# baldhat/yolov10-3D

Hardware: AMD Instinct MI355X
Metric: train_images_per_sec (higher is better)
Workload: dtype bf16

## Files before the change

### include/y3d.h

```cpp
#ifndef Y3D_H
#define Y3D_H
#include <stdint.h>

#ifdef __cplusplus
extern "C" {
#endif

enum { Y3D_F32 = 0, Y3D_BF16 = 1 };
enum { Y3D_OK = 0, Y3D_ERR_INVALID = -1, Y3D_ERR_HIP = -2 };

const char* y3d_last_error(void);
int y3d_abi_version(void);
int y3d_device_info(char* name, int name_len, int* compute_units, int* lds_bytes, int* clock_khz);

int y3d_pack_weight_fwd(int dtype, const float* w_oihw, void* out, int Cout, int Cin_g, int Cin_g_pad, int kh, int kw, void* stream);
int y3d_pack_weight_dgrad(int dtype, const float* w_oihw, void* out, int Cout, int Cin_g, int groups, int kh, int kw, void* stream);
int y3d_mt_pack_weights(int dtype, const int64_t* desc, const int* chunk_tensor, const int* chunk_off, int nchunks, int chunk, void* stream);
int y3d_mt_fp8w_quantize(const int64_t* desc, const int* row_begin, int ntensors, int nrows, void* stream);
int y3d_fp8w_dequantize(const uint8_t* codes, const float* scale, float* w, int rows, int K, void* stream);
int y3d_fp8_quantize_act(const void* x, int64_t xsw, int64_t M, int C, uint8_t* q, uint8_t* s, void* stream);
int y3d_fp8_pack_weight_fwd(const uint8_t* codes, const float* scale, int rows, int Cg, uint8_t* wq, uint8_t* ws, void* stream);
int y3d_conv3x3_fp8_ok(int B, int H, int W, int Cin, int Cout, int groups);
int y3d_conv3x3_fp8_stat_rows(int B, int H, int W);
int y3d_fp8_scale_pitch(int C);
// ... 13 lines not shown
  Y3D_ROUTE_GENERIC = 0,
  Y3D_ROUTE_STREAM1X1 = 1,
  Y3D_ROUTE_SMALL = 2,
  Y3D_ROUTE_SMALL_S2 = 3,
  Y3D_ROUTE_S2_DGRAD = 4,
  Y3D_ROUTE_TILE8 = 5,
  Y3D_ROUTE_TILE16 = 6,
  Y3D_ROUTE_WIDE3_8 = 7,
  Y3D_ROUTE_WIDE3_16 = 8,
  Y3D_ROUTE_FLAT = 9,
  Y3D_ROUTE_WGRAD_SMALL = 10,
  Y3D_ROUTE_WGRAD_TILE = 11,
  Y3D_ROUTE_WGRAD_STREAM1X1 = 12
};
int y3d_conv2d_route(int dtype, int op, int epi, int B, int H, int W, int Cin, int Cout, int groups, int kh, int kw, int stride, int pad);
int y3d_conv2d_fwd(int dtype, const void* x, int64_t xsb, int64_t xsh, int64_t xsw, int B, int H, int W, int Cin,
                   const void* w_packed, const float* bias, void* y, int64_t ysw, int Ho, int Wo, int Cout, int groups,
                   int kh, int kw, int stride, int pad, float* stat_partials, void* stream);
int y3d_conv2d_fwd_affine(int dtype, const void* x, int64_t xsb, int64_t xsh, int64_t xsw, int B, int H, int W, int Cin,
                          const void* w_packed, const float* scale, const float* shift, int act, void* y, int64_t ysw, int Ho, int Wo,
                          int Cout, int groups, int kh, int kw, int stride, int pad, void* stream);
int y3d_conv2d_fwd_affine_res_ok(int dtype, int B, int H, int W, int Cin, int Cout, int groups, int kh, int kw, int stride, int pad);
int y3d_conv2d_fwd_affine_res(int dtype, const void* x, int64_t xsb, int64_t xsh, int64_t xsw, int B, int H, int W, int Cin,
                              const void* w_packed, const float* scale, const float* shift, int act, const void* res, int64_t rsw, void* y,
                              int64_t ysw, int Ho, int Wo, int Cout, int groups, int kh, int kw, int stride, int pad, void* stream);
int y3d_conv2d_bwd_data(int dtype, const void* dy, int64_t dsb, int64_t dsh, int64_t dsw, int B, int Ho, int Wo, int Cout,
                        const void* w_packed_dgrad, void* dx, int64_t xsw, int H, int W, int Cin, int groups, int kh, int kw,
                        int stride, int pad, void* stream);
int y3d_conv2d_wgrad_splits(int dtype, int B, int Ho, int Wo, int Cout, int Cin_g, int groups, int kh, int kw);
int y3d_conv2d_wgrad_plan(int dtype, int B, int H, int W, int Cin, int Cout, int groups, int kh, int kw, int stride, int pad);
int y3d_set_tile_kernels(int enable);
int y3d_set_stream1x1(int enable);
int y3d_get_stream1x1(void);
int y3d_get_tile_kernels(void);
int y3d_set_bn_wide_slabs(int enable);
int y3d_conv2d_bwd_weight(int dtype, const void* x, int64_t xsb, int64_t xsh, int64_t xsw, int B, int H, int W, int Cin,
                          int Cin_real, const void* dy, int64_t dsw, int Ho, int Wo, int Cout, int groups, int kh, int kw,
                          int stride, int pad, float* slab, int nsplit, float* grad_oihw, int accumulate, void* stream);

int y3d_dw_blocks(int64_t M);
int y3d_dw_wgrad_blocks(int64_t M);
int y3d_dw_pack_weight(const float* w_oihw, float* out_taps_c, int C, int kh, int kw, void* stream);
int y3d_dwconv2d_fwd(int dtype, const void* x, int64_t xsb, int64_t xsh, int64_t xsw, int B, int H, int W, int C,
                     const float* w_packed, void* y, int64_t ysw, int Ho, int Wo, int kh, int kw, int stride, int pad,
                     float* stat_partials, void* stream);
int y3d_dwconv2d_fwd_affine(int dtype, const void* x, int64_t xsb, int64_t xsh, int64_t xsw, int B, int H, int W, int C,
                            const float* w_packed, const float* scale, const float* shift, int act, int res_mode, const void* res, int64_t rsw,
                            void* z, int64_t zsw, int Ho, int Wo, int kh, int kw, int stride, int pad, void* stream);
int y3d_dwconv2d_bwd_data(int dtype, const void* dy, int64_t dsb, int64_t dsh, int64_t dsw, int B, int Ho, int Wo, int C,
                          const float* w_packed, void* dx, int64_t xsw, int H, int W, int kh, int kw, int stride, int pad,
                          void* stream);
int y3d_dwconv2d_bwd_weight(int dtype, const void* x, int64_t xsb, int64_t xsh, int64_t xsw, int B, int H, int W, int C,
                            const void* dy, int64_t dsw, int Ho, int Wo, int kh, int kw, int stride, int pad, float* slab,
                            float* grad_oihw, int accumulate, void* stream);

int y3d_bn_finalize(const float* partials, int nblk, int C, int64_t count, const float* gamma, const float* beta, float eps,
                    float momentum, float* running_mean, float* running_var, float* mean, float* invstd, float* scale,
                    float* shift, void* stream);
int y3d_bn_eval_scale(int C, const float* gamma, const float* beta, const float* running_mean, const float* running_var,
                      float eps, float* scale, float* shift, void* stream);
int y3d_bn_act_fwd(int dtype, const void* y, int64_t ysw, const float* scale, const float* shift, int act, int res_mode,
                   const void* res, int64_t rsw, void* z, int64_t zsw, int64_t P, int C, void* stream);
int y3d_bn_act_fwd_q(const void* y, int64_t ysw, const float* scale, const float* shift, int act, void* z, int64_t zsw, uint8_t* q, uint8_t* s,
                     int64_t P, int C, void* stream);
int y3d_bn_bwd_blocks(int64_t P, int C);
int y3d_bn_act_bwd_reduce(int dtype, const void* y, int64_t ysw, const void* dz, int64_t dsw, const void* res, int64_t rsw,
// ... 192 lines not shown
```

### yolov10-3d_amd/_lib.py

```python
from __future__ import annotations

import ctypes
import os
import re

_HERE = os.path.dirname(os.path.abspath(__file__))
LIB_PATH = os.path.join(_HERE, "liby3d_hip.so")
HEADER = os.path.join(os.path.dirname(_HERE), "include", "y3d.h")

F32, BF16 = 0, 1

_CT = {"int": ctypes.c_int, "int64_t": ctypes.c_int64, "float": ctypes.c_float, "double": ctypes.c_double}


class Y3DError(RuntimeError):
    pass


def parse_header(path: str = HEADER):
    src = open(path).read()
    src = re.sub(r"/\*.*?\*/", " ", src, flags=re.S)
    protos = {}
    for m in re.finditer(r"(const\s+char\s*\*|int)\s+(y3d_\w+)\s*\(([^;{]*?)\)\s*;", src, flags=re.S):
        ret, name, args = m.group(1), m.group(2), m.group(3).strip()
        argtypes = []
        if args and args != "void":
            for a in args.split(","):
                a = a.strip()
                if "*" in a:
                    argtypes.append(ctypes.c_void_p)
                else:
                    toks = a.split()
                    t = toks[1] if toks[0] == "const" else toks[0]
                    argtypes.append(_CT[t])
        protos[name] = (ctypes.c_char_p if "char" in ret else ctypes.c_int, argtypes)
    return protos


_PLAIN_INT = {"abi_version", "conv_kpad", "conv_stat_blocks", "conv2d_stat_rows", "conv2d_route", "conv2d_wgrad_splits", "conv2d_wgrad_plan", "set_tile_kernels", "set_stream1x1", "set_bn_wide_slabs", "get_stream1x1", "get_tile_kernels", "dw_blocks", "dw_wgrad_blocks", "bn_bwd_blocks", "proj_blocks", "proj_group_blocks", "proj_group_bn_bwd_blocks", "proj_group_bwd_weight_bn_mfma_blocks", "tal3d_scratch_floats", "tal2d_scratch_floats", "v10_postprocess_scratch_floats", "conv2d_fwd_affine_res_ok", "stem_conv_train_rows", "conv3x3_fp8_ok", "conv3x3_fp8_dgrad_ok", "conv3x3_fp8_stat_rows", "fp8_scale_pitch", "kitti_eval_max_boxes", "det_metrics_max_gts", "det_metrics_max_dets"}


class _Lib:
    def __init__(self):
        if not os.path.exists(LIB_PATH):
            raise Y3DError(
                f"{LIB_PATH} not found: build it with `python yolov10-3d_amd/csrc/build.py` "
                "(or __graft_entry__.build()). There is no CPU / PyTorch fallback for the HIP path.")
        self._dll = ctypes.CDLL(LIB_PATH)
        self.protos = parse_header()
        for name, (ret, argtypes) in self.protos.items():
            fn = getattr(self._dll, name)
            fn.restype = ret
            fn.argtypes = argtypes

    def last_error(self) -> str:
        return (self._dll.y3d_last_error() or b"").decode()

    def __getattr__(self, name):
        if name.startswith("_"):
            raise AttributeError(name)
        fn = getattr(self._dll, "y3d_" + name)
        ret = self.protos["y3d_" + name][0]
        if ret is not ctypes.c_int or name in _PLAIN_INT:
            setattr(self, name, fn)
            return fn

        def call(*a):
            rc = fn(*a)
            if rc != 0:
                raise Y3DError(f"y3d_{name} failed ({rc}): {self.last_error()}")
            return rc

# ... 13 lines not shown
```

### yolov10-3d_amd/csrc/conv1x1_stream.hip

```cpp
#include "common.h"
#include "conv_frag.h"
#include <cstdlib>

namespace {

struct PwP {
  const bf16_t* x;
  const bf16_t* w;
  const float *bias, *scale, *shift;
  bf16_t* y;
  float* part;
  long ysw;
  int xsw;
  int M, K, N, Kpad;
  int nkc, nmt, nnt, act;
  int G, PC;
  unsigned xbytes, ybytes, pbytes, wbytes;
};

template <int N> __device__ __forceinline__ void pw_wvm() { asm volatile("s_waitcnt vmcnt(%0)" ::"n"(N) : "memory"); }
__device__ __forceinline__ void pw_wvm_n(int n) {
#define PW_C(i) case i: pw_wvm<i>(); break;
#define PW_C8(i) PW_C(i) PW_C(i + 1) PW_C(i + 2) PW_C(i + 3) PW_C(i + 4) PW_C(i + 5) PW_C(i + 6) PW_C(i + 7)
  switch (n) {
    PW_C8(0) PW_C8(8) PW_C8(16) PW_C8(24) PW_C8(32) PW_C8(40) PW_C8(48) PW_C(56) PW_C(57) PW_C(58) PW_C(59) PW_C(60) PW_C(61) PW_C(62)
    default: pw_wvm<63>(); break;
  }
#undef PW_C8
#undef PW_C
}
typedef __attribute__((ext_vector_type(2))) unsigned pw_u32x2;

template <int BN, int WP, int WC, int NS, bool AFF, bool WRES>
__global__ __launch_bounds__(512) void conv1x1_stream_kernel(PwP p) {
  {
    const int g = blockIdx.y;
    p.x += (long)g * p.K;
    p.w += (long)g * p.N * p.Kpad;
    p.y += (long)g * p.N;
    if (p.bias) p.bias += g * p.N;
    if (p.scale) { p.scale += g * p.N; p.shift += g * p.N; }
    if (p.part) p.part += (long)g * p.N * 2;
  }
  constexpr int BM = 128;
  constexpr int TP = BM / WP / 16, TC = BN / WC / 16;
  static_assert(WP * WC == 8 && TP >= 1 && TC >= 1, "8 waves");
  constexpr int STAGE = BM * 128 + (WRES ? 0 : BN * 128);
  constexpr int ND = 2 + (WRES ? 0 : BN / 64);
  static_assert(WRES || BN % 64 == 0, "streamed weight tiles: whole DMA instructions per wave");
  extern __shared__ __attribute__((aligned(16))) char smem[];
  char* sW = smem;
  char* sA = smem + (WRES ? (size_t)p.nkc * BN * 128 : 0);
  const int tid = threadIdx.x, lane = tid & 63, wave = __builtin_amdgcn_readfirstlane(tid >> 6);
  const int wp = wave % WP, wc = wave / WP;
  const int bid = blockIdx.x, xcd = bid & 7, idx = bid >> 3;
  const int nt = idx % p.nnt, wk = (idx / p.nnt) * 8 + xcd, nwk = (gridDim.x / p.nnt);
  const int n0 = nt * BN;
  const int mine = wk < p.nmt ? (p.nmt - wk + nwk - 1) / nwk : 0;
  const int S = mine * p.nkc;
  if (S == 0) {
    if (p.part && tid < BN && n0 + tid < p.N) *(float2*)(p.part + ((long)wk * p.PC + n0 + tid) * 2) = make_float2(0.f, 0.f);
    return;
  }

  if (WRES)
  for (int i = tid; i < p.nkc * BN * 8; i += 512) {
    const int c = i & 7, r = (i >> 3) % BN, kc = i / (8 * BN);
    const int k = kc * 64 + c * 8, n = n0 + r;
    uint4 v = make_uint4(0, 0, 0, 0);
    if (n < p.N && k < p.Kpad) v = *(const uint4*)(p.w + (long)n * p.Kpad + k);
    *(uint4*)(sW + (kc * BN + r) * 128 + ((c ^ (r & 7)) << 4)) = v;
  }

  const __amdgpu_buffer_rsrc_t rx = __builtin_amdgcn_make_buffer_rsrc((void*)p.x, 0, (int)p.xbytes, 0x00020000);
  const __amdgpu_buffer_rsrc_t rw = __builtin_amdgcn_make_buffer_rsrc((void*)p.w, 0, (int)p.wbytes, 0x00020000);
  constexpr unsigned OOB = 0xfffffff0u;
  const int lrow = lane >> 3, lchunk = (lane & 7) ^ lrow;
  int is = 0, i_tile = wk, i_kc = 0, i_slot = 0;
  auto issue = [&]() {
    const bool live = is < S;
    const int k = i_kc * 64 + lchunk * 8;
#pragma unroll
    for (int h = 0; h < 2; ++h) {
      const int r = 16 * wave + 8 * h;
      const int m = i_tile * BM + r + lrow;
      const bool ok = live & (m < p.M) & (k < p.K);
      const unsigned off = (unsigned)(m * p.xsw + k) * 2u;
      __builtin_amdgcn_raw_ptr_buffer_load_lds(rx, (__attribute__((address_space(3))) void*)(sA + i_slot * STAGE + r * 128), 16, ok ? off : OOB, 0, 0, 0);
    }
    if (!WRES) {
#pragma unroll
      for (int h = 0; h < BN / 64; ++h) {
        const int r = (BN / 8) * wave + 8 * h;
        const int n = n0 + r + lrow;
        const bool ok = live & (n < p.N) & (k < p.K);
        __builtin_amdgcn_raw_ptr_buffer_load_lds(rw, (__attribute__((address_space(3))) void*)(sA + i_slot * STAGE + (BM + r) * 128), 16,
                                                 ok ? (unsigned)(n * p.Kpad + k) * 2u : OOB, 0, 0, 0);
      }
    }
    ++is;
    if (++i_kc == p.nkc) { i_kc = 0; i_tile += nwk; }
    if (++i_slot == NS) i_slot = 0;
  };
#pragma unroll
  for (int s = 0; s < NS - 1; ++s) issue();

  f32x4_t acc[TC][TP];
  const int lc = (lane >> 4) * 4, lp = lane & 15;
  int c_tile = wk, c_kc = 0, c_slot = 0;
  int hist[NS - 1];
#pragma unroll
  for (int i = 0; i < NS - 1; ++i) hist[i] = 0;
  const __amdgpu_buffer_rsrc_t ry = __builtin_amdgcn_make_buffer_rsrc((void*)p.y, 0, (int)p.ybytes, 0x00020000);
  asm volatile("s_waitcnt lgkmcnt(0)" ::: "memory");

  float ssum[TC][4], ssq[TC][4];
#pragma unroll
  for (int a = 0; a < TC; ++a)
#pragma unroll
    for (int j = 0; j < 4; ++j) { ssum[a][j] = 0.f; ssq[a][j] = 0.f; }

#pragma unroll 1
  for (int s = 0; s < S; ++s) {
    {
      int young = ND * (NS - 2);
#pragma unroll
      for (int i = 0; i < NS - 1; ++i) young += hist[i];
      pw_wvm_n(young);
#pragma unroll
      for (int i = 0; i < NS - 2; ++i) hist[i] = hist[i + 1];
      hist[NS - 2] = 0;
    }
    __builtin_amdgcn_s_barrier();
    issue();
    if (c_kc == 0) {
#pragma unroll
      for (int a = 0; a < TC; ++a)
#pragma unroll
// ... 48 lines not shown
      }
    }
    hist[NS - 2] += TC * TP;
    c_tile += nwk;
  }
  pw_wvm<0>();
  if (p.part) {
    __syncthreads();
    float* red = (float*)sA;
#pragma unroll
    for (int a = 0; a < TC; ++a)
#pragma unroll
      for (int j = 0; j < 4; ++j) {
        const float s = wave_xor_sum16(ssum[a][j]), q = wave_xor_sum16(ssq[a][j]);
        if (lp == 0) {
          const int cl = wc * (BN / WC) + a * 16 + lc + j;
          red[(wp * BN + cl) * 2] = s;
          red[(wp * BN + cl) * 2 + 1] = q;
        }
      }
    __syncthreads();
    if (tid < BN && n0 + tid < p.N) {
      float s = 0.f, q = 0.f;
#pragma unroll
      for (int w = 0; w < WP; ++w) { s += red[(w * BN + tid) * 2]; q += red[(w * BN + tid) * 2 + 1]; }
      float* dst = p.part + ((long)wk * p.PC + n0 + tid) * 2;
      dst[0] = s;
      dst[1] = q;
    }
  }
}

struct PwPlan {
  int bn, ns, nnt, grid, wres;
  size_t lds;
};

bool pw_plan(int M, int K, int N, PwPlan* pl, int G = 1) {
  const int nkc = cdiv(K, 64);
  const size_t cap = 160 * 1024;
  const int nmt = cdiv(M, 128);
  const int bns[4] = {256, 128, 64, 32};
  int bn = 0;
  for (int i = 0; i < 4; ++i) {
    const int b = bns[i];
    if (i < 3 && bns[i + 1] >= N) continue;
    if ((size_t)b * nkc * 128 + 3 * 16384 <= cap) { bn = b; break; }
  }
  const bool can_stream = N > 64 && nkc >= 2;
  bool wres = bn != 0 && (cdiv(N, bn) == 1 || (cdiv(N, bn) == 2 && nmt < 200));
  if (!wres && !can_stream) {
    if (!bn) return false;
    wres = true;
  }
  pl->wres = wres;
  if (wres) {
    const size_t wb = (size_t)bn * nkc * 128;
    pl->bn = bn;
    pl->ns = wb + 4 * 16384 <= cap ? 4 : 3;
    pl->lds = wb + pl->ns * 16384;
  } else {
    pl->bn = N > 128 ? 256 : 128;
    pl->ns = pl->bn == 256 ? 3 : 4;
    pl->lds = (size_t)pl->ns * (16384 + pl->bn * 128);
  }
  pl->nnt = cdiv(N, pl->bn);
  const int per_cu = pl->lds <= 80 * 1024 ? 2 : 1;
  int wpx = (32 * per_cu) / (pl->nnt * G);
  if (wpx < 1) wpx = 1;
  if (wpx > cdiv(nmt, 8)) wpx = cdiv(nmt, 8);
  pl->grid = 8 * wpx * pl->nnt;
  return true;
}

template <int BN, int WP, int WC, int NS, bool AFF, bool WRES>
void pw_launch_1(const PwP& p, const PwPlan& pl, hipStream_t st) {
  static bool attr = false;
  if (!attr) {
    (void)hipFuncSetAttribute((const void*)conv1x1_stream_kernel<BN, WP, WC, NS, AFF, WRES>, hipFuncAttributeMaxDynamicSharedMemorySize, 160 * 1024);
    attr = true;
  }
  hipLaunchKernelGGL((conv1x1_stream_kernel<BN, WP, WC, NS, AFF, WRES>), dim3(pl.grid, p.G), dim3(512), pl.lds, st, p);
}

template <int BN, int WP, int WC>
void pw_launch_ns(const PwP& p, const PwPlan& pl, hipStream_t st) {
  const bool aff = p.bias || p.scale;
  if (pl.ns == 4) { if (aff) pw_launch_1<BN, WP, WC, 4, true, true>(p, pl, st); else pw_launch_1<BN, WP, WC, 4, false, true>(p, pl, st); }
  else { if (aff) pw_launch_1<BN, WP, WC, 3, true, true>(p, pl, st); else pw_launch_1<BN, WP, WC, 3, false, true>(p, pl, st); }
}

}

static int g_stream1x1 = 1;

extern "C" int y3d_get_stream1x1(void) { return g_stream1x1; }

extern "C" int y3d_set_stream1x1(int enable) {
  const int old = g_stream1x1;
  g_stream1x1 = enable ? 1 : 0;
  return old;
}

int y3d_conv1x1_stream_ok(int dtype, long M, int K, int N, long xsw, int G) {
  if (!g_stream1x1 || dtype != Y3D_BF16 || K % 8 != 0 || K < 32 || N < 8 || N % 4 != 0 || M < 128 || G < 1 || G > 64) return 0;
  if ((M * xsw + (long)G * K) * 2 >= (1L << 32) - 64 || M * N * G * 2 >= (1L << 31)) return 0;
  PwPlan pl;
  if (!pw_plan((int)M, K, N, &pl, G)) return 0;
  return 1;
}

int y3d_conv1x1_stream_rows(long M, int K, int N, int G) {
  PwPlan pl;
  if (!pw_plan((int)M, K, N, &pl, G)) return 0;
  return pl.grid / pl.nnt;
}

int y3d_conv1x1_stream_launch(const void* x, long xsw, const void* w, int Kpad, const float* bias, const float* scale, const float* shift, int act,
                              void* y, long ysw, float* part, long M, int K, int N, int G, void* stream) {
  PwPlan pl;
  Y3D_CHECK(pw_plan((int)M, K, N, &pl, G), "conv1x1_stream: no tile plan for K=%d N=%d", K, N);
  Y3D_CHECK(((uintptr_t)x & 15) == 0 && xsw % 8 == 0 && ((uintptr_t)w & 15) == 0 && Kpad % 8 == 0 && ((uintptr_t)y & 7) == 0 && ysw % 4 == 0,
            "conv1x1_stream: operand alignment");
  PwP p;
  p.x = (const bf16_t*)x; p.w = (const bf16_t*)w; p.bias = bias; p.scale = scale; p.shift = shift; p.y = (bf16_t*)y; p.part = part;
  p.ysw = ysw; p.xsw = (int)xsw; p.M = (int)M; p.K = K; p.N = N; p.Kpad = Kpad;
  p.nkc = cdiv(K, 64); p.nmt = cdiv(M, 128); p.nnt = pl.nnt; p.act = act; p.G = G; p.PC = G * N;
  p.xbytes = (unsigned)(((M - 1) * xsw + K) * 2);
  Y3D_CHECK(((M - 1) * ysw + (long)G * N) * 2 < (1L << 32) - 64 && M * ysw < (1L << 31), "conv1x1_stream: output tensor beyond 32-bit byte offsets");
  p.ybytes = (unsigned)(((M - 1) * ysw + N) * 2);
  p.pbytes = part ? (unsigned)((long)p.nmt * N * 8) : 0u;
  hipStream_t st = (hipStream_t)stream;
  p.wbytes = (unsigned)((long)N * Kpad * 2);
  if (!pl.wres) {
    const bool aff = bias || scale;
    if (pl.bn == 256) { if (aff) pw_launch_1<256, 2, 4, 3, true, false>(p, pl, st); else pw_launch_1<256, 2, 4, 3, false, false>(p, pl, st); }
    else { if (aff) pw_launch_1<128, 4, 2, 4, true, false>(p, pl, st); else pw_launch_1<128, 4, 2, 4, false, false>(p, pl, st); }
    Y3D_LAUNCH_CHECK();
    return Y3D_OK;
  }
  switch (pl.bn) {
    case 256: pw_launch_ns<256, 2, 4>(p, pl, st); break;
    case 128: pw_launch_ns<128, 4, 2>(p, pl, st); break;
    case 64: pw_launch_ns<64, 8, 1>(p, pl, st); break;
    default: pw_launch_ns<32, 8, 1>(p, pl, st); break;
  }
  Y3D_LAUNCH_CHECK();
  return Y3D_OK;
}
```

### yolov10-3d_amd/csrc/conv_gemm.hip

```cpp
#include "common.h"
#include "conv_frag.h"
#include <cstdlib>

namespace {

struct ConvP {
  const void* x;
  const void* w;
  const float* bias;
  const float* scale;
  const float* shift;
  int act;
  void* y;
  float* part;
  long xsb, xsh, xsw;
  long ysw;
  int B, Hg, Wg;
  int Hq, Wq;
  int Cg, Cn, G;
  int kh, kw, stride, pad;
  int Ktot, Kpad;
  int M;
  int ntx, nty;
};
// ... 635 lines not shown
    size_t sm = 2 * (128 + 64) * 128;
    hipLaunchKernelGGL((conv_gemm_kernel<T, 128, 64, 4, 1, MODE>), dim3(p.ntx * p.nty, ny, p.G), block, sm, st, p);
  } else {
    size_t sm = 2 * (128 + 32) * 128;
    hipLaunchKernelGGL((conv_gemm_kernel<T, 128, 32, 4, 1, MODE>), dim3(p.ntx * p.nty, ny, p.G), block, sm, st, p);
  }
  Y3D_LAUNCH_CHECK();
  return Y3D_OK;
}

template <typename T, bool DGRAD>
int launch_conv(ConvP p, hipStream_t st) {
  if (DGRAD && p.kh == 3 && p.kw == 3 && p.stride == 2 && p.pad == 1 && p.Cg % TT<T>::CE == 0) return launch_conv_mode<T, 2>(p, st);
  return launch_conv_mode<T, DGRAD ? 1 : 0>(p, st);
}

}

int y3d_conv3x3_tile_route(int dtype, int B, int H, int W, int Cg, int Cn, int G, int kh, int kw, int stride, int pad);
int y3d_conv3x3_flat_tiles(int B, int H, int W);
int y3d_conv3x3_tile_launch(int dtype, int route, const void* x, long xsb, long xsh, long xsw, int B, int H, int W, int Cg, int Cn, int G,
                            const void* w, int Ktot, void* y, long ysw, float* part, int flip, const float* scale, const float* shift, int act,
                            void* stream);

int y3d_wgrad_tile_height(int dtype, int H, int W, int Cg, int Cn, int kh, int kw, int stride, int pad);
int y3d_wgrad_tile_splits(int th, int B, int H, int W, int Cg, int Cn, int G);
int y3d_conv3x3_wgrad_tile_launch(int th, const void* x, long xsb, long xsh, long xsw, const void* dy, long dsw, int B, int H, int W, int Cg,
                                  int Cn, int G, float* slab, int nsplit, void* stream);

int y3d_conv1x1_stream_ok(int dtype, long M, int K, int N, long xsw, int G = 1);
int y3d_conv1x1_stream_launch(const void* x, long xsw, const void* w, int Kpad, const float* bias, const float* scale, const float* shift, int act,
                              void* y, long ysw, float* part, long M, int K, int N, int G, void* stream);
int y3d_wgrad1x1_stream_ok(int dtype, long M, int Cg, int Cn, long xsw, long dsw);
int y3d_wgrad1x1_stream_launch(const void* x, long xsw, const void* dy, long dsw, long M, int Cg, int Cn, float* slab, int nsplit, int chunk_px,
                               void* stream);
int y3d_conv3x3s2_dgrad_ok(int dtype, int B, int Ho, int Wo, int H, int W, int Cout, int Cin, long dsw, long xsw);
int y3d_conv3x3s2_dgrad_launch(const void* dy, long dsw, int B, int Ho, int Wo, int Cout, const void* w_packed_dgrad, int Kpad, void* dx, long xsw,
                               int H, int W, int Cin, void* stream);
int y3d_conv3x3_small_ok(int dtype, int B, int H, int W, int Cin, int Cout, int rows);
int y3d_conv3x3_small_launch(const void* x, long xsb, long xsh, long xsw, int B, int H, int W, int Cin, int Cout, const void* w, int Ktot, void* y,
                             long ysw, float* part, int rows, int flip, const float* scale, const float* shift, int act, const void* res, long rsw,
                             void* stream);
int y3d_conv3x3_small_rows(int B, int H, int W, int Cin, int Cout);
int y3d_conv3x3_small_s2_ok(int dtype, int B, int H, int W, int Cin, int Cout);
int y3d_conv3x3_small_s2_rows(int B, int H, int W, int Cin, int Cout);
int y3d_conv3x3_small_s2_launch(const void* x, long xsb, long xsh, long xsw, int B, int H, int W, int Cin, int Cout, const void* w, int Ktot, void* y,
                                long ysw, float* part, int rows, const float* scale, const float* shift, int act, void* stream);
int y3d_conv1x1_stream_rows(long M, int K, int N, int G = 1);
int y3d_wgrad3x3_small_ok(int dtype, int B, int H, int W, int Cin, int Cout);
int y3d_wgrad3x3_small_splits(int B, int H, int W);
int y3d_wgrad3x3_small_launch(const void* x, long xsb, long xsh, long xsw, const void* dy, long dsw, int B, int H, int W, int Cin, int Cout,
                              float* slab, int nsplit, void* stream);
static inline bool dense_pixels(int B, int H, int W, long sb, long sh, long sw) {
  return (H == 1 || sh == (long)W * sw) && (B == 1 || sb == (long)H * W * sw);
}

static int g_tile_kernels = 1;
extern "C" int y3d_conv2d_wgrad_splits(int dtype, int B, int Ho, int Wo, int Cout, int Cin_g, int groups, int kh, int kw);

static int conv_route(int dtype, int op, int epi, int B, int H, int W, int Ho, int Wo, int Cin, int Cout, int groups, int kh, int kw, int stride,
                      int pad, bool dense, long asw, long bsw, bool cin_full) {
  const int ce = dtype == Y3D_BF16 ? 8 : 4;
  const bool k1 = kh == 1 && kw == 1 && stride == 1 && pad == 0, k3s1 = kh == 3 && kw == 3 && stride == 1 && pad == 1,
             k3s2 = kh == 3 && kw == 3 && stride == 2 && pad == 1;
  if (op == Y3D_OP_FWD) {
    Y3D_CHECK(dtype == Y3D_BF16 || dtype == Y3D_F32, "conv2d_fwd: bad dtype %d", dtype);
// ... 35 lines not shown
  if (k3s1 && groups == 1 && cin_full && y3d_wgrad3x3_small_ok(dtype, B, H, W, Cin, Cout)) return Y3D_ROUTE_WGRAD_SMALL;
  if (g_tile_kernels && cin_full && y3d_wgrad_tile_height(dtype, H, W, Cin / groups, Cout / groups, kh, kw, stride, pad)) return Y3D_ROUTE_WGRAD_TILE;
  if (k1 && groups == 1 && cin_full && dense && y3d_wgrad1x1_stream_ok(dtype, (long)B * Ho * Wo, Cin, Cout, asw, bsw)) return Y3D_ROUTE_WGRAD_STREAM1X1;
  return Y3D_ROUTE_GENERIC;
}

extern "C" {

int y3d_get_tile_kernels(void) { return g_tile_kernels; }

int y3d_set_tile_kernels(int enable) {
  int old = g_tile_kernels;
  g_tile_kernels = enable ? 1 : 0;
  return old;
}

int y3d_conv_stat_blocks(int B, int Ho, int Wo) { return cdiv((long)B * Ho * Wo, 128); }

int y3d_conv2d_route(int dtype, int op, int epi, int B, int H, int W, int Cin, int Cout, int groups, int kh, int kw, int stride, int pad) {
  Y3D_CHECK(kh > 0 && kw > 0 && stride > 0 && pad >= 0, "conv2d_route: bad filter geometry");
  const int Ho = (H + 2 * pad - kh) / stride + 1, Wo = (W + 2 * pad - kw) / stride + 1;
  Y3D_CHECK(Ho > 0 && Wo > 0, "conv2d_route: empty output");
  if (op == Y3D_OP_BWD_DATA) return conv_route(dtype, op, epi, B, H, W, Ho, Wo, Cin, Cout, groups, kh, kw, stride, pad, true, Cout, Cin, true);
  return conv_route(dtype, op, epi, B, H, W, Ho, Wo, Cin, Cout, groups, kh, kw, stride, pad, true, Cin, Cout, true);
}

int y3d_conv2d_wgrad_plan(int dtype, int B, int H, int W, int Cin, int Cout, int groups, int kh, int kw, int stride, int pad) {
  int Ho = (H + 2 * pad - kh) / stride + 1, Wo = (W + 2 * pad - kw) / stride + 1;
  switch (conv_route(dtype, Y3D_OP_BWD_WEIGHT, 0, B, H, W, Ho, Wo, Cin, Cout, groups, kh, kw, stride, pad, true, Cin, Cout, true)) {
    case Y3D_ROUTE_WGRAD_SMALL: return y3d_wgrad3x3_small_splits(B, H, W);
    case Y3D_ROUTE_WGRAD_TILE:
      return y3d_wgrad_tile_splits(y3d_wgrad_tile_height(dtype, H, W, Cin / groups, Cout / groups, kh, kw, stride, pad), B, H, W, Cin / groups,
                                   Cout / groups, groups);
    case Y3D_ROUTE_WGRAD_STREAM1X1: {
      const int target = 256;
      const long tiles = (long)cdiv(Cin, Cin <= 64 ? 64 : 128) * cdiv(Cout, Cout <= 64 ? 64 : 128);
      long want = target / tiles, maxs = cdiv((long)B * H * W, 4 * 64);
      if (want > maxs) want = maxs;
      return (int)(want < 1 ? 1 : want);
    }
    default: return y3d_conv2d_wgrad_splits(dtype, B, Ho, Wo, Cout, Cin / groups, groups, kh, kw);
  }
}

int y3d_conv2d_stat_rows(int dtype, int B, int H, int W, int Cin, int Cout, int groups, int kh, int kw, int stride, int pad) {
  int Ho = (H + 2 * pad - kh) / stride + 1, Wo = (W + 2 * pad - kw) / stride + 1;
  switch (conv_route(dtype, Y3D_OP_FWD, Y3D_EPI_PARTIALS, B, H, W, Ho, Wo, Cin, Cout, groups, kh, kw, stride, pad, true, Cin, Cout, true)) {
    case Y3D_ROUTE_STREAM1X1: return y3d_conv1x1_stream_rows((long)B * H * W, Cin / groups, Cout / groups, groups);
    case Y3D_ROUTE_SMALL: return y3d_conv3x3_small_rows(B, H, W, Cin, Cout);
    case Y3D_ROUTE_SMALL_S2: return y3d_conv3x3_small_s2_rows(B, H, W, Cin, Cout);
    case Y3D_ROUTE_FLAT: return y3d_conv3x3_flat_tiles(B, H, W);
    case Y3D_ROUTE_TILE8: case Y3D_ROUTE_WIDE3_8: return B * cdiv(H, 8) * cdiv(W, 16);
    case Y3D_ROUTE_TILE16: case Y3D_ROUTE_WIDE3_16: return B * cdiv(H, 16) * cdiv(W, 16);
    default: return cdiv((long)B * Ho * Wo, 128);
  }
}

int y3d_conv_kpad(int dtype, int k_total) {
  int ce = dtype == Y3D_BF16 ? 8 : 4;
  return cdiv(k_total, ce) * ce;
}

int y3d_pack_weight_fwd(int dtype, const float* w_oihw, void* out, int Cout, int Cin_g, int Cin_g_pad, int kh, int kw, void* stream) {
  int ce = dtype == Y3D_BF16 ? 8 : 4;
  Y3D_CHECK(Cin_g_pad >= Cin_g && Cin_g_pad % ce == 0, "pack_weight_fwd: Cin_g_pad=%d must be a multiple of %d", Cin_g_pad, ce);
  int taps = kh * kw, Kpad = taps * Cin_g_pad;
  long n = (long)Cout * Kpad;
  hipStream_t st = (hipStream_t)stream;
  if (dtype == Y3D_BF16)
    hipLaunchKernelGGL(pack_w_fwd_kernel<bf16_t>, dim3(cdiv(n, 256)), dim3(256), 0, st, w_oihw, (bf16_t*)out, Cout, Cin_g, Cin_g_pad, taps, Kpad);
  else
    hipLaunchKernelGGL(pack_w_fwd_kernel<float>, dim3(cdiv(n, 256)), dim3(256), 0, st, w_oihw, (float*)out, Cout, Cin_g, Cin_g_pad, taps, Kpad);
  Y3D_LAUNCH_CHECK();
// ... 221 lines not shown
```

### yolov10-3d_amd/csrc/wgrad1x1_stream.hip

```cpp
#include "common.h"

namespace {

struct Wg1P {
  const bf16_t* x;
  const bf16_t* dy;
  float* slab;
  int xsw, dsw;
  int M, Cg, Cn, chunk_px;
  unsigned xbytes, dbytes;
};

template <int N> __device__ __forceinline__ void wg1_wvm() { asm volatile("s_waitcnt vmcnt(%0)" ::"n"(N) : "memory"); }

__device__ __forceinline__ s16x4_t wg1_tr(unsigned a) {
  s16x4_t v;
  asm volatile("ds_read_b64_tr_b16 %0, %1" : "=v"(v) : "v"(a));
  return v;
}
template <int NF>
__device__ __forceinline__ void wg1_wait(s16x4_t (&f)[NF][2]) {
  if constexpr (NF == 2) asm volatile("s_waitcnt lgkmcnt(0)" : "+v"(f[0][0]), "+v"(f[0][1]), "+v"(f[1][0]), "+v"(f[1][1]));
  else if constexpr (NF == 3) asm volatile("s_waitcnt lgkmcnt(0)" : "+v"(f[0][0]), "+v"(f[0][1]), "+v"(f[1][0]), "+v"(f[1][1]), "+v"(f[2][0]), "+v"(f[2][1]));
  else if constexpr (NF == 4) asm volatile("s_waitcnt lgkmcnt(0)" : "+v"(f[0][0]), "+v"(f[0][1]), "+v"(f[1][0]), "+v"(f[1][1]), "+v"(f[2][0]), "+v"(f[2][1]), "+v"(f[3][0]), "+v"(f[3][1]));
// ... 96 lines not shown
      for (int a = 0; a < TA; ++a)
#pragma unroll
        for (int b = 0; b < TB; ++b) acc[a][b] = __builtin_amdgcn_mfma_f32_16x16x32_bf16(fr[a], fr[TA + b], acc[a][b], 0, 0, 0);
    }
    if (++c_slot == NS) c_slot = 0;
  }
  wg1_wvm<0>();
  float* slab = p.slab + (long)split * p.Cn * p.Cg;
#pragma unroll
  for (int a = 0; a < TA; ++a)
#pragma unroll
    for (int b = 0; b < TB; ++b) {
      const int k = j0 + wj * (WX / WXW) + b * 16 + li;
#pragma unroll
      for (int r = 0; r < 4; ++r) {
        const int co = i0 + wi * (WD / WDW) + a * 16 + grp * 4 + r;
        if (co < p.Cn && k < p.Cg) slab[(long)co * p.Cg + k] = acc[a][b][r];
      }
    }
}

template <int WD, int WX, int WDW>
void wg1_launch(const Wg1P& p, dim3 grid, hipStream_t st) {
  constexpr int CD = WD / 8 + 2, CX = WX / 8 + 2;
  const size_t lds = (size_t)4 * 64 * (CD + CX) * 16 + 1024;
  static bool attr = false;
  if (!attr) {
    (void)hipFuncSetAttribute((const void*)wgrad1x1_stream_kernel<WD, WX, WDW>, hipFuncAttributeMaxDynamicSharedMemorySize, 160 * 1024);
    attr = true;
  }
  hipLaunchKernelGGL((wgrad1x1_stream_kernel<WD, WX, WDW>), grid, dim3(512), lds, st, p);
}

}

extern "C" int y3d_get_stream1x1(void);

int y3d_wgrad1x1_stream_ok(int dtype, long M, int Cg, int Cn, long xsw, long dsw) {
  if (!y3d_get_stream1x1() || dtype != Y3D_BF16 || Cg <= 32 || Cn <= 32 || Cg % 8 || Cn % 8) return 0;
  if ((M * xsw + Cg) * 2 >= (1L << 32) - 64 || (M * dsw + Cn) * 2 >= (1L << 32) - 64) return 0;
  return 1;
}

int y3d_wgrad1x1_stream_launch(const void* x, long xsw, const void* dy, long dsw, long M, int Cg, int Cn, float* slab, int nsplit, int chunk_px,
                               void* stream) {
  Wg1P p;
  p.x = (const bf16_t*)x; p.dy = (const bf16_t*)dy; p.slab = slab; p.xsw = (int)xsw; p.dsw = (int)dsw;
  p.M = (int)M; p.Cg = Cg; p.Cn = Cn; p.chunk_px = chunk_px;
  p.xbytes = (unsigned)(((M - 1) * xsw + Cg) * 2);
  p.dbytes = (unsigned)(((M - 1) * dsw + Cn) * 2);
  const int wd = Cn <= 64 ? 64 : 128, wx = Cg <= 64 ? 64 : 128;
  dim3 grid(cdiv(Cg, wx), cdiv(Cn, wd), nsplit);
  hipStream_t st = (hipStream_t)stream;
  if (wd == 128 && wx == 128) wg1_launch<128, 128, 2>(p, grid, st);
  else if (wd == 64 && wx == 128) wg1_launch<64, 128, 2>(p, grid, st);
  else if (wd == 128 && wx == 64) wg1_launch<128, 64, 4>(p, grid, st);
  else wg1_launch<64, 64, 2>(p, grid, st);
  Y3D_LAUNCH_CHECK();
  return Y3D_OK;
}
```

Baseline: 1404.

## Add shape-tuned small-tile variants for 1x1 conv forward and weight-grad stream kernels

Templates the 1x1 conv stream kernel on the M tile size (64 or 128) and adds alternative tile and staging variants, picked from per-shape tables keyed on M, K and N for the low-resolution layers. The 1x1 weight-grad kernel gets similar per-shape plans that choose smaller output tiles and recompute the split count to match. The aim is more parallelism and better CU occupancy on small-M layers, where the default 128-wide tiles leave the GPU underfilled. It adds more template instantiations and a shape-specific dispatch that only helps the listed shapes.

```diff
diff --git a/include/y3d.h b/include/y3d.h
--- a/include/y3d.h
+++ b/include/y3d.h
@@ -69,6 +69,10 @@
 int y3d_set_tile_kernels(int enable);
 int y3d_set_stream1x1(int enable);
 int y3d_get_stream1x1(void);
+int y3d_set_conv1x1_small(int mode);
+int y3d_conv1x1_stream_plan(int M, int K, int N, int groups, int* out);
+int y3d_set_wgrad1x1_small(int mode);
+int y3d_wgrad1x1_stream_plan(int M, int Cin, int Cout, int* out);
 int y3d_get_tile_kernels(void);
 int y3d_set_bn_wide_slabs(int enable);
 int y3d_conv2d_bwd_weight(int dtype, const void* x, int64_t xsb, int64_t xsh, int64_t xsw, int B, int H, int W, int Cin,
diff --git a/yolov10-3d_amd/_lib.py b/yolov10-3d_amd/_lib.py
--- a/yolov10-3d_amd/_lib.py
+++ b/yolov10-3d_amd/_lib.py
@@ -37,7 +37,7 @@
     return protos
 
 
-_PLAIN_INT = {"abi_version", "conv_kpad", "conv_stat_blocks", "conv2d_stat_rows", "conv2d_route", "conv2d_wgrad_splits", "conv2d_wgrad_plan", "set_tile_kernels", "set_stream1x1", "set_bn_wide_slabs", "get_stream1x1", "get_tile_kernels", "dw_blocks", "dw_wgrad_blocks", "bn_bwd_blocks", "proj_blocks", "proj_group_blocks", "proj_group_bn_bwd_blocks", "proj_group_bwd_weight_bn_mfma_blocks", "tal3d_scratch_floats", "tal2d_scratch_floats", "v10_postprocess_scratch_floats", "conv2d_fwd_affine_res_ok", "stem_conv_train_rows", "conv3x3_fp8_ok", "conv3x3_fp8_dgrad_ok", "conv3x3_fp8_stat_rows", "fp8_scale_pitch", "kitti_eval_max_boxes", "det_metrics_max_gts", "det_metrics_max_dets"}
+_PLAIN_INT = {"abi_version", "conv_kpad", "conv_stat_blocks", "conv2d_stat_rows", "conv2d_route", "conv2d_wgrad_splits", "conv2d_wgrad_plan", "set_tile_kernels", "set_stream1x1", "set_conv1x1_small", "conv1x1_stream_plan", "wgrad1x1_stream_plan", "set_wgrad1x1_small", "set_bn_wide_slabs", "get_stream1x1", "get_tile_kernels", "dw_blocks", "dw_wgrad_blocks", "bn_bwd_blocks", "proj_blocks", "proj_group_blocks", "proj_group_bn_bwd_blocks", "proj_group_bwd_weight_bn_mfma_blocks", "tal3d_scratch_floats", "tal2d_scratch_floats", "v10_postprocess_scratch_floats", "conv2d_fwd_affine_res_ok", "stem_conv_train_rows", "conv3x3_fp8_ok", "conv3x3_fp8_dgrad_ok", "conv3x3_fp8_stat_rows", "fp8_scale_pitch", "kitti_eval_max_boxes", "det_metrics_max_gts", "det_metrics_max_dets"}
 
 
 class _Lib:
diff --git a/yolov10-3d_amd/csrc/conv1x1_stream.hip b/yolov10-3d_amd/csrc/conv1x1_stream.hip
--- a/yolov10-3d_amd/csrc/conv1x1_stream.hip
+++ b/yolov10-3d_amd/csrc/conv1x1_stream.hip
@@ -31,7 +31,7 @@
 }
 typedef __attribute__((ext_vector_type(2))) unsigned pw_u32x2;
 
-template <int BN, int WP, int WC, int NS, bool AFF, bool WRES>
+template <int BM, int BN, int WP, int WC, int NS, bool AFF, bool WRES>
 __global__ __launch_bounds__(512) void conv1x1_stream_kernel(PwP p) {
   {
     const int g = blockIdx.y;
@@ -42,11 +42,11 @@
     if (p.scale) { p.scale += g * p.N; p.shift += g * p.N; }
     if (p.part) p.part += (long)g * p.N * 2;
   }
-  constexpr int BM = 128;
   constexpr int TP = BM / WP / 16, TC = BN / WC / 16;
   static_assert(WP * WC == 8 && TP >= 1 && TC >= 1, "8 waves");
+  static_assert(BM == 128 || BM == 64, "whole 8-row DMA instructions per wave");
   constexpr int STAGE = BM * 128 + (WRES ? 0 : BN * 128);
-  constexpr int ND = 2 + (WRES ? 0 : BN / 64);
+  constexpr int ND = BM / 64 + (WRES ? 0 : BN / 64);
   static_assert(WRES || BN % 64 == 0, "streamed weight tiles: whole DMA instructions per wave");
   extern __shared__ __attribute__((aligned(16))) char smem[];
   char* sW = smem;
@@ -63,14 +63,16 @@
     return;
   }
 
-  if (WRES)
-  for (int i = tid; i < p.nkc * BN * 8; i += 512) {
-    const int c = i & 7, r = (i >> 3) % BN, kc = i / (8 * BN);
-    const int k = kc * 64 + c * 8, n = n0 + r;
-    uint4 v = make_uint4(0, 0, 0, 0);
-    if (n < p.N && k < p.Kpad) v = *(const uint4*)(p.w + (long)n * p.Kpad + k);
-    *(uint4*)(sW + (kc * BN + r) * 128 + ((c ^ (r & 7)) << 4)) = v;
-  }
+  auto load_weights = [&]() {
+    if (WRES)
+    for (int i = tid; i < p.nkc * BN * 8; i += 512) {
+      const int c = i & 7, r = (i >> 3) % BN, kc = i / (8 * BN);
+      const int k = kc * 64 + c * 8, n = n0 + r;
+      uint4 v = make_uint4(0, 0, 0, 0);
+      if (n < p.N && k < p.Kpad) v = *(const uint4*)(p.w + (long)n * p.Kpad + k);
+      *(uint4*)(sW + (kc * BN + r) * 128 + ((c ^ (r & 7)) << 4)) = v;
+    }
+  };
 
   const __amdgpu_buffer_rsrc_t rx = __builtin_amdgcn_make_buffer_rsrc((void*)p.x, 0, (int)p.xbytes, 0x00020000);
   const __amdgpu_buffer_rsrc_t rw = __builtin_amdgcn_make_buffer_rsrc((void*)p.w, 0, (int)p.wbytes, 0x00020000);
@@ -81,8 +83,8 @@
     const bool live = is < S;
     const int k = i_kc * 64 + lchunk * 8;
 #pragma unroll
-    for (int h = 0; h < 2; ++h) {
-      const int r = 16 * wave + 8 * h;
+    for (int h = 0; h < BM / 64; ++h) {
+      const int r = (BM / 8) * wave + 8 * h;
       const int m = i_tile * BM + r + lrow;
       const bool ok = live & (m < p.M) & (k < p.K);
       const unsigned off = (unsigned)(m * p.xsw + k) * 2u;
@@ -102,8 +104,10 @@
     if (++i_kc == p.nkc) { i_kc = 0; i_tile += nwk; }
     if (++i_slot == NS) i_slot = 0;
   };
+  if (BM == 128) load_weights();
 #pragma unroll
   for (int s = 0; s < NS - 1; ++s) issue();
+  if (BM != 128) load_weights();
 
   f32x4_t acc[TC][TP];
   const int lc = (lane >> 4) * 4, lp = lane & 15;
@@ -218,11 +222,15 @@
 }
 
 struct PwPlan {
-  int bn, ns, nnt, grid, wres;
+  int bm, bn, ns, nnt, grid, wres, variant;
+  int wp;
   size_t lds;
 };
 
-bool pw_plan(int M, int K, int N, PwPlan* pl, int G = 1) {
+enum { PW_BASE = 0, PW_S256 = 1, PW_R128 = 2, PW_S128 = 3, PW_R64 = 4, PW_S128W = 5, PW_NVARIANTS = 6 };
+static int g_small1x1 = 0;
+
+bool pw_plan_base(int M, int K, int N, PwPlan* pl, int G) {
   const int nkc = cdiv(K, 64);
   const size_t cap = 160 * 1024;
   const int nmt = cdiv(M, 128);
@@ -239,6 +247,8 @@
     if (!bn) return false;
     wres = true;
   }
+  pl->bm = 128;
+  pl->variant = PW_BASE;
   pl->wres = wres;
   if (wres) {
     const size_t wb = (size_t)bn * nkc * 128;
@@ -259,21 +269,109 @@
   return true;
 }
 
-template <int BN, int WP, int WC, int NS, bool AFF, bool WRES>
+bool pw_plan_small(int variant, int M, int K, int N, PwPlan* pl, int G) {
+  if (G != 1) return false;
+  const int nkc = cdiv(K, 64);
+  const size_t cap = 160 * 1024;
+  pl->bm = variant == PW_S128W ? 128 : 64;
+  const int nmt = cdiv(M, pl->bm);
+  pl->variant = variant;
+  switch (variant) {
+    case PW_S256:
+      if (N <= 128) return false;
+      pl->bn = 256; pl->wres = 0; pl->ns = 4; pl->lds = (size_t)4 * (8192 + 256 * 128);
+      break;
+    case PW_S128:
+      if (N <= 64) return false;
+      pl->bn = 128; pl->wres = 0; pl->ns = 4; pl->lds = (size_t)4 * (8192 + 128 * 128);
+      break;
+    case PW_S128W:
+      if (N <= 128) return false;
+      pl->bn = 128; pl->wres = 0; pl->ns = 4; pl->lds = (size_t)4 * (16384 + 128 * 128);
+      break;
+    case PW_R128: case PW_R64: {
+      const int bn = variant == PW_R128 ? 128 : 64;
+      if (variant == PW_R128 && N <= 64) return false;
+      const size_t wb = (size_t)bn * nkc * 128;
+      if (wb + 3 * 8192 > cap) return false;
+      pl->bn = bn; pl->wres = 1; pl->ns = wb + 4 * 8192 <= cap ? 4 : 3; pl->lds = wb + pl->ns * 8192;
+      break;
+    }
+    default: return false;
+  }
+  pl->nnt = cdiv(N, pl->bn);
+  const int per_cu = pl->lds <= 80 * 1024 ? 2 : 1;
+  int wpx = (32 * per_cu) / pl->nnt;
+  if (wpx < 1) wpx = 1;
+  if (wpx > cdiv(nmt, 8)) wpx = cdiv(nmt, 8);
+  pl->grid = 8 * wpx * pl->nnt;
+  return true;
+}
+
+struct PwSmallRow { int K, N, variant; };
+const PwSmallRow pw_small20[] = {{512, 256, PW_S128W}, {256, 256, PW_S128W}};
+const PwSmallRow pw_small40[] = {{256, 384, PW_S128W}};
+
+int pw_small_variant(int M, int K, int N, int G) {
+  if (G != 1) return PW_BASE;
+  const PwSmallRow* rows = nullptr;
+  int n = 0;
+  if (M > 6400 && M <= 12800) { rows = pw_small20; n = sizeof(pw_small20) / sizeof(PwSmallRow); }
+  else if (M > 25600 && M <= 51200) { rows = pw_small40; n = sizeof(pw_small40) / sizeof(PwSmallRow); }
+  for (int i = 0; i < n; ++i)
+    if (rows[i].K == K && rows[i].N == N) return rows[i].variant;
+  return PW_BASE;
+}
+
+bool pw_plan(int M, int K, int N, PwPlan* pl, int G = 1) {
+  PwPlan base;
+  if (!pw_plan_base(M, K, N, &base, G)) return false;
+  const int v = g_small1x1 > 0 ? g_small1x1 : g_small1x1 == 0 ? pw_small_variant(M, K, N, G) : PW_BASE;
+  if (v == PW_BASE || !pw_plan_small(v, M, K, N, pl, G)) *pl = base;
+  pl->wp = base.bn == 256 ? 2 : 4;
+  return true;
+}
+
+template <int BM, int BN, int WP, int WC, int NS, bool AFF, bool WRES>
 void pw_launch_1(const PwP& p, const PwPlan& pl, hipStream_t st) {
   static bool attr = false;
   if (!attr) {
-    (void)hipFuncSetAttribute((const void*)conv1x1_stream_kernel<BN, WP, WC, NS, AFF, WRES>, hipFuncAttributeMaxDynamicSharedMemorySize, 160 * 1024);
+    (void)hipFuncSetAttribute((const void*)conv1x1_stream_kernel<BM, BN, WP, WC, NS, AFF, WRES>, hipFuncAttributeMaxDynamicSharedMemorySize, 160 * 1024);
     attr = true;
   }
-  hipLaunchKernelGGL((conv1x1_stream_kernel<BN, WP, WC, NS, AFF, WRES>), dim3(pl.grid, p.G), dim3(512), pl.lds, st, p);
-}
-
-template <int BN, int WP, int WC>
+  hipLaunchKernelGGL((conv1x1_stream_kernel<BM, BN, WP, WC, NS, AFF, WRES>), dim3(pl.grid, p.G), dim3(512), pl.lds, st, p);
+}
+
+template <int BM, int BN, int WP, int WC>
 void pw_launch_ns(const PwP& p, const PwPlan& pl, hipStream_t st) {
   const bool aff = p.bias || p.scale;
-  if (pl.ns == 4) { if (aff) pw_launch_1<BN, WP, WC, 4, true, true>(p, pl, st); else pw_launch_1<BN, WP, WC, 4, false, true>(p, pl, st); }
-  else { if (aff) pw_launch_1<BN, WP, WC, 3, true, true>(p, pl, st); else pw_launch_1<BN, WP, WC, 3, false, true>(p, pl, st); }
+  if (pl.ns == 4) { if (aff) pw_launch_1<BM, BN, WP, WC, 4, true, true>(p, pl, st); else pw_launch_1<BM, BN, WP, WC, 4, false, true>(p, pl, st); }
+  else { if (aff) pw_launch_1<BM, BN, WP, WC, 3, true, true>(p, pl, st); else pw_launch_1<BM, BN, WP, WC, 3, false, true>(p, pl, st); }
+}
+
+void pw_launch_small(const PwP& p, const PwPlan& pl, hipStream_t st) {
+  const bool aff = p.bias || p.scale;
+  switch (pl.variant) {
+    case PW_S256:
+      if (aff) pw_launch_1<64, 256, 2, 4, 4, true, false>(p, pl, st); else pw_launch_1<64, 256, 2, 4, 4, false, false>(p, pl, st);
+      break;
+    case PW_S128:
+      if (aff) pw_launch_1<64, 128, 2, 4, 4, true, false>(p, pl, st); else pw_launch_1<64, 128, 2, 4, 4, false, false>(p, pl, st);
+      break;
+    case PW_R128:
+      pw_launch_ns<64, 128, 2, 4>(p, pl, st);
+      break;
+    case PW_S128W:
+      if (pl.wp == 2) {
+        if (aff) pw_launch_1<128, 128, 2, 4, 4, true, false>(p, pl, st); else pw_launch_1<128, 128, 2, 4, 4, false, false>(p, pl, st);
+      } else {
+        if (aff) pw_launch_1<128, 128, 4, 2, 4, true, false>(p, pl, st); else pw_launch_1<128, 128, 4, 2, 4, false, false>(p, pl, st);
+      }
+      break;
+    default:
+      pw_launch_ns<64, 64, 4, 2>(p, pl, st);
+      break;
+  }
 }
 
 }
@@ -286,6 +384,25 @@
   const int old = g_stream1x1;
   g_stream1x1 = enable ? 1 : 0;
   return old;
+}
+
+extern "C" int y3d_set_conv1x1_small(int mode) {
+  const int old = g_small1x1;
+  g_small1x1 = mode < -1 || mode >= PW_NVARIANTS ? 0 : mode;
+  return old;
+}
+
+int y3d_conv1x1_stream_ok(int dtype, long M, int K, int N, long xsw, int G);
+
+extern "C" int y3d_conv1x1_stream_plan(int M, int K, int N, int groups, int* out) {
+  PwPlan pl;
+  if (!y3d_conv1x1_stream_ok(Y3D_BF16, M, K, N, (long)K * groups, groups)) return -1;
+  if (!pw_plan(M, K, N, &pl, groups)) return -1;
+  if (out) {
+    const int v[8] = {pl.variant, pl.bm, pl.bn, pl.ns, pl.nnt, pl.grid, pl.wres, (int)pl.lds};
+    for (int i = 0; i < 8; ++i) out[i] = v[i];
+  }
+  return pl.variant;
 }
 
 int y3d_conv1x1_stream_ok(int dtype, long M, int K, int N, long xsw, int G) {
@@ -311,25 +428,30 @@
   PwP p;
   p.x = (const bf16_t*)x; p.w = (const bf16_t*)w; p.bias = bias; p.scale = scale; p.shift = shift; p.y = (bf16_t*)y; p.part = part;
   p.ysw = ysw; p.xsw = (int)xsw; p.M = (int)M; p.K = K; p.N = N; p.Kpad = Kpad;
-  p.nkc = cdiv(K, 64); p.nmt = cdiv(M, 128); p.nnt = pl.nnt; p.act = act; p.G = G; p.PC = G * N;
+  p.nkc = cdiv(K, 64); p.nmt = cdiv(M, pl.bm); p.nnt = pl.nnt; p.act = act; p.G = G; p.PC = G * N;
   p.xbytes = (unsigned)(((M - 1) * xsw + K) * 2);
   Y3D_CHECK(((M - 1) * ysw + (long)G * N) * 2 < (1L << 32) - 64 && M * ysw < (1L << 31), "conv1x1_stream: output tensor beyond 32-bit byte offsets");
   p.ybytes = (unsigned)(((M - 1) * ysw + N) * 2);
   p.pbytes = part ? (unsigned)((long)p.nmt * N * 8) : 0u;
   hipStream_t st = (hipStream_t)stream;
   p.wbytes = (unsigned)((long)N * Kpad * 2);
+  if (pl.variant != PW_BASE) {
+    pw_launch_small(p, pl, st);
+    Y3D_LAUNCH_CHECK();
+    return Y3D_OK;
+  }
   if (!pl.wres) {
     const bool aff = bias || scale;
-    if (pl.bn == 256) { if (aff) pw_launch_1<256, 2, 4, 3, true, false>(p, pl, st); else pw_launch_1<256, 2, 4, 3, false, false>(p, pl, st); }
-    else { if (aff) pw_launch_1<128, 4, 2, 4, true, false>(p, pl, st); else pw_launch_1<128, 4, 2, 4, false, false>(p, pl, st); }
+    if (pl.bn == 256) { if (aff) pw_launch_1<128, 256, 2, 4, 3, true, false>(p, pl, st); else pw_launch_1<128, 256, 2, 4, 3, false, false>(p, pl, st); }
+    else { if (aff) pw_launch_1<128, 128, 4, 2, 4, true, false>(p, pl, st); else pw_launch_1<128, 128, 4, 2, 4, false, false>(p, pl, st); }
     Y3D_LAUNCH_CHECK();
     return Y3D_OK;
   }
   switch (pl.bn) {
-    case 256: pw_launch_ns<256, 2, 4>(p, pl, st); break;
-    case 128: pw_launch_ns<128, 4, 2>(p, pl, st); break;
-    case 64: pw_launch_ns<64, 8, 1>(p, pl, st); break;
-    default: pw_launch_ns<32, 8, 1>(p, pl, st); break;
+    case 256: pw_launch_ns<128, 256, 2, 4>(p, pl, st); break;
+    case 128: pw_launch_ns<128, 128, 4, 2>(p, pl, st); break;
+    case 64: pw_launch_ns<128, 64, 8, 1>(p, pl, st); break;
+    default: pw_launch_ns<128, 32, 8, 1>(p, pl, st); break;
   }
   Y3D_LAUNCH_CHECK();
   return Y3D_OK;
diff --git a/yolov10-3d_amd/csrc/conv_gemm.hip b/yolov10-3d_amd/csrc/conv_gemm.hip
--- a/yolov10-3d_amd/csrc/conv_gemm.hip
+++ b/yolov10-3d_amd/csrc/conv_gemm.hip
@@ -691,6 +691,7 @@
 int y3d_conv1x1_stream_launch(const void* x, long xsw, const void* w, int Kpad, const float* bias, const float* scale, const float* shift, int act,
                               void* y, long ysw, float* part, long M, int K, int N, int G, void* stream);
 int y3d_wgrad1x1_stream_ok(int dtype, long M, int Cg, int Cn, long xsw, long dsw);
+int y3d_wgrad1x1_stream_splits(long M, int Cg, int Cn);
 int y3d_wgrad1x1_stream_launch(const void* x, long xsw, const void* dy, long dsw, long M, int Cg, int Cn, float* slab, int nsplit, int chunk_px,
                                void* stream);
 int y3d_conv3x3s2_dgrad_ok(int dtype, int B, int Ho, int Wo, int H, int W, int Cout, int Cin, long dsw, long xsw);
@@ -792,13 +793,7 @@
     case Y3D_ROUTE_WGRAD_TILE:
       return y3d_wgrad_tile_splits(y3d_wgrad_tile_height(dtype, H, W, Cin / groups, Cout / groups, kh, kw, stride, pad), B, H, W, Cin / groups,
                                    Cout / groups, groups);
-    case Y3D_ROUTE_WGRAD_STREAM1X1: {
-      const int target = 256;
-      const long tiles = (long)cdiv(Cin, Cin <= 64 ? 64 : 128) * cdiv(Cout, Cout <= 64 ? 64 : 128);
-      long want = target / tiles, maxs = cdiv((long)B * H * W, 4 * 64);
-      if (want > maxs) want = maxs;
-      return (int)(want < 1 ? 1 : want);
-    }
+    case Y3D_ROUTE_WGRAD_STREAM1X1: return y3d_wgrad1x1_stream_splits((long)B * H * W, Cin, Cout);
     default: return y3d_conv2d_wgrad_splits(dtype, B, Ho, Wo, Cout, Cin / groups, groups, kh, kw);
   }
 }
diff --git a/yolov10-3d_amd/csrc/wgrad1x1_stream.hip b/yolov10-3d_amd/csrc/wgrad1x1_stream.hip
--- a/yolov10-3d_amd/csrc/wgrad1x1_stream.hip
+++ b/yolov10-3d_amd/csrc/wgrad1x1_stream.hip
@@ -152,9 +152,60 @@
   hipLaunchKernelGGL((wgrad1x1_stream_kernel<WD, WX, WDW>), grid, dim3(512), lds, st, p);
 }
 
+enum { WG1_WIDE = 0, WG1_64x64 = 1, WG1_64x128 = 2, WG1_NPLANS = 3 };
+int g_wgrad_small = 0;
+
+struct Wg1Row { int Cg, Cn, plan; };
+const Wg1Row wg1_small20[] = {{512, 256, WG1_64x128}, {256, 512, WG1_64x128}, {768, 512, WG1_64x128}, {256, 256, WG1_64x64}};
+const Wg1Row wg1_small40[] = {{256, 512, WG1_64x128}, {512, 256, WG1_64x128}};
+
+int wg1_plan(long M, int Cg, int Cn) {
+  if (g_wgrad_small < 0 || M > 51200) return WG1_WIDE;
+  if (g_wgrad_small > 0) return g_wgrad_small;
+  const Wg1Row* rows = nullptr;
+  int n = 0;
+  if (M > 6400 && M <= 12800) { rows = wg1_small20; n = sizeof(wg1_small20) / sizeof(Wg1Row); }
+  else if (M > 25600) { rows = wg1_small40; n = sizeof(wg1_small40) / sizeof(Wg1Row); }
+  for (int i = 0; i < n; ++i)
+    if (rows[i].Cg == Cg && rows[i].Cn == Cn) return rows[i].plan;
+  return WG1_WIDE;
+}
+
+void wg1_tile(int plan, int Cg, int Cn, int* wd, int* wx) {
+  *wd = plan != WG1_WIDE || Cn <= 64 ? 64 : 128;
+  *wx = plan == WG1_64x64 || Cg <= 64 ? 64 : 128;
+}
+
 }
 
 extern "C" int y3d_get_stream1x1(void);
+
+extern "C" int y3d_set_wgrad1x1_small(int mode) {
+  const int old = g_wgrad_small;
+  g_wgrad_small = mode < -1 || mode >= WG1_NPLANS ? 0 : mode;
+  return old;
+}
+
+int y3d_wgrad1x1_stream_splits(long M, int Cg, int Cn);
+extern "C" int y3d_wgrad1x1_stream_plan(int M, int Cg, int Cn, int* out) {
+  const int plan = wg1_plan(M, Cg, Cn);
+  if (out) {
+    int wd, wx;
+    wg1_tile(plan, Cg, Cn, &wd, &wx);
+    out[0] = plan; out[1] = wd; out[2] = wx; out[3] = cdiv(Cg, wx) * cdiv(Cn, wd); out[4] = y3d_wgrad1x1_stream_splits(M, Cg, Cn);
+  }
+  return plan;
+}
+
+int y3d_wgrad1x1_stream_splits(long M, int Cg, int Cn) {
+  const int plan = wg1_plan(M, Cg, Cn);
+  int wd, wx;
+  wg1_tile(plan, Cg, Cn, &wd, &wx);
+  const long tiles = (long)cdiv(Cg, wx) * cdiv(Cn, wd);
+  long want = 256 / tiles, maxs = plan == WG1_WIDE ? cdiv(M, 4 * 64) : M / (8 * 64);
+  if (want > maxs) want = maxs;
+  return (int)(want < 1 ? 1 : want);
+}
 
 int y3d_wgrad1x1_stream_ok(int dtype, long M, int Cg, int Cn, long xsw, long dsw) {
   if (!y3d_get_stream1x1() || dtype != Y3D_BF16 || Cg <= 32 || Cn <= 32 || Cg % 8 || Cn % 8) return 0;
@@ -169,7 +220,8 @@
   p.M = (int)M; p.Cg = Cg; p.Cn = Cn; p.chunk_px = chunk_px;
   p.xbytes = (unsigned)(((M - 1) * xsw + Cg) * 2);
   p.dbytes = (unsigned)(((M - 1) * dsw + Cn) * 2);
-  const int wd = Cn <= 64 ? 64 : 128, wx = Cg <= 64 ? 64 : 128;
+  int wd, wx;
+  wg1_tile(wg1_plan(M, Cg, Cn), Cg, Cn, &wd, &wx);
   dim3 grid(cdiv(Cg, wx), cdiv(Cn, wd), nsplit);
   hipStream_t st = (hipStream_t)stream;
   if (wd == 128 && wx == 128) wg1_launch<128, 128, 2>(p, grid, st);
```

Result: no change. 1412, median of 3 (+0.5%).
